# Li-Jinjie/ndp_nmpc_qd

Hardware: AMD Instinct MI355X
Metric: NMPC solves/sec (N=20, 1 RTI iter + downwash MLP) at batch (higher is better)
Workload: dtype f64

## Files before the change

### ndp_nmpc_qd_amd/build.py

```python
import os
import subprocess
import sys
from concurrent.futures import ThreadPoolExecutor

HERE = os.path.dirname(os.path.abspath(__file__))
CSRC = os.path.join(HERE, "csrc")
LIB = os.path.join(HERE, "libndp_nmpc_hip.so")
UNITS = ["ndp_hip.hip", "exchange.hip", "mlp_vjp.hip"]
HEADERS = sorted(f for f in os.listdir(CSRC) if f.endswith((".hpp", ".inc"))) + [os.path.join("..", "..", "include", "ndp_nmpc.h")]
FLAGS = ["--offload-arch=gfx950", "-O3", "-std=c++17", "-mllvm", "-amdgpu-mfma-vgpr-form",
         "-mllvm", "-amdgpu-schedule-relaxed-occupancy=true", "-fPIC"]


def _mtime(p):
    return os.path.getmtime(p) if os.path.exists(p) else -1.0


def build(force=False, verbose=False, out=LIB, extra=()):
    flags = FLAGS + os.environ.get("NDP_EXTRA_HIPCC_FLAGS", "").split() + list(extra)
    odir = os.path.join(HERE, "build", os.path.splitext(os.path.basename(out))[0])
    os.makedirs(odir, exist_ok=True)
    stamp = os.path.join(odir, "flags")
    if not os.path.exists(stamp) or open(stamp).read() != " ".join(flags):
        force = True
    t_hdr = max(_mtime(os.path.join(CSRC, f)) for f in HEADERS)
    objs = [os.path.join(odir, os.path.splitext(u)[0] + ".o") for u in UNITS]
    todo = [(u, o) for u, o in zip(UNITS, objs) if force or _mtime(o) < max(t_hdr, _mtime(os.path.join(CSRC, u)))]

    def compile_unit(job):
        u, o = job
        cmd = ["hipcc"] + flags + ["-c", "-o", o, os.path.join(CSRC, u)]
        if verbose:
            print(" ".join(cmd), flush=True)
        return subprocess.run(cmd, cwd=CSRC).returncode

    if todo:
        if os.path.exists(stamp):
            os.remove(stamp)
        jobs = max(1, min(16, len(todo), int(os.environ.get("MAX_JOBS") or 16)))
        with ThreadPoolExecutor(jobs) as ex:
            failed = [u for (u, _), rc in zip(todo, ex.map(compile_unit, todo)) if rc != 0]
        if failed:
            raise subprocess.CalledProcessError(1, "hipcc " + " ".join(failed))
        with open(stamp, "w") as fh:
            fh.write(" ".join(flags))
    if todo or _mtime(out) < max(_mtime(o) for o in objs):
        cmd = ["hipcc", "-shared", "-o", out] + objs
        if verbose:
            print(" ".join(cmd), flush=True)
        subprocess.check_call(cmd, cwd=CSRC)
    return out


if __name__ == "__main__":
    args = sys.argv[1:]
    out = LIB
    if args[:1] == ["-o"]:
        out, args = os.path.abspath(args[1]), args[2:]
    print(build(force=True, verbose=True, out=out, extra=args))
```

### ndp_nmpc_qd_amd/csrc/kern_args.hpp

```cpp
#pragma once
#include <hip/hip_runtime.h>

#include <stddef.h>

namespace ndp {

struct ThrCfg { double a1, a2, hm, g, R, Q0, Q1, mass; };

struct RingGeom {
    int step, np1;
    __host__ __device__ int ring() const { return step * (np1 - 1) + 1; }
    __host__ __device__ size_t px() const { return (size_t)step * 2 * np1 * 10; }
    __host__ __device__ size_t pu() const { return (size_t)step * 2 * np1 * 4; }
    __host__ __device__ size_t slot(unsigned long long j) const { return (size_t)(j % step) * 2 * np1 + (size_t)((j / step) % np1); }
};

struct RefCfg { int B, N, n_seg; double dt, mass, g, toff; };

struct TickPre {
    RefCfg cf;
    const double *coeff, *tcum, *tseg, *fpt;
    int *seg_hint;
    const double *t;
    double t_all;
    int advance;
    unsigned long long j_new;
    RingGeom rg;
    double *rx, *ru;
    ThrCfg thr;
    double *st;
// ... 10 lines not shown
```

### ndp_nmpc_qd_amd/csrc/ndp_hip.hip

```cpp
#include <hip/hip_runtime.h>
#include <hip/hip_ext.h>

#include <sched.h>
#include <stdio.h>

#include <atomic>
#include <chrono>
#include <condition_variable>
#include <cstdlib>
#include <cstring>
#include <memory>
#include <mutex>
#include <new>
#include <string>
#include <thread>
#include <type_traits>
#include <vector>

#include "wave_gfx950.hpp"
#include "cfg_params.hpp"
#include "cond_qp.hpp"
#include "host.hpp"
#include "mlp_common.hpp"

namespace ndp {

struct BatchPtrs {
    const double *kc;
    const int *tables;
    const double *x0, *xr, *ur;
    const float *f;
    double *X, *U, *u0;
    int *status, *iters;
    double *Xm, *Um;
    double *dbg;
    double *stamps;
    size_t xr_pitch, ur_pitch;
    size_t x0_pitch;
    double *cmd;
    const double *kthr;
    double *thrust_keep;
    double cmd_mass;
    int f_f64;
    signed char *act;
};

struct MlpArgs {
    const float *frag;
    const double *other;
    const double *ego_xy;
    float *force_out;
    double r2;
    int other_stride;
// ... 3 lines not shown
    size_t ego_pitch;
};

struct QueueArgs {
    unsigned *count;
    int *ids;
    unsigned long long *ipm_total;
};

typedef __attribute__((address_space(3))) float *lds_f32;
typedef const __attribute__((address_space(3))) float *lds_cf32;
__device__ __forceinline__ void stage_fragments(const float *__restrict__ fr, lds_f32 dst, int tid, int nthreads);
__device__ __forceinline__ void mlp_tile(lds_cf32 fr, const float zb[3], int lane, float o[3]);
__device__ __forceinline__ bool gate_open(const double *other_inst, const double *ego_xy_inst, double r2);

__device__ __forceinline__ void bind_instance(RtiIo &io, const BatchPtrs &bp, int inst, int N)
{
    const size_t nx = (size_t)(N + 1) * NX, nu = (size_t)N * NU, nf = (size_t)(N + 1) * 3;
    io.x0 = bp.x0 + (size_t)inst * bp.x0_pitch;
    io.xr = bp.xr + inst * bp.xr_pitch;
    io.ur = bp.ur + inst * bp.ur_pitch;
    io.f = bp.f ? bp.f + inst * nf * (bp.f_f64 ? 2 : 1) : nullptr;
    io.f_is_f64 = bp.f_f64;
    io.X = bp.X + inst * nx;
    io.U = bp.U + inst * nu;
    io.Xm = bp.Xm ? bp.Xm + inst * nx : nullptr;
    io.Um = bp.Xm ? bp.Um + inst * nu : nullptr;
    io.u0 = bp.u0 + (size_t)inst * NU;
    io.status = bp.status + inst;
    io.iters = bp.iters + inst;
    io.dbg = bp.dbg;
    io.f_in_lds = 0;
    io.kc = bp.kc;
    io.tables = bp.tables;
    io.stamps = bp.stamps ? bp.stamps + (size_t)inst * NDP_NSTAMP : nullptr;
    io.act = bp.act ? bp.act + (size_t)inst * act_pitch(N) : nullptr;
    if (NDP_RARELY(bp.cmd != nullptr)) {
        io.cmd = bp.cmd + (size_t)inst * NU;
        io.thrust_keep = bp.thrust_keep + inst;
        io.kthr = bp.kthr[inst];
// ... 50 lines not shown
    LateArgs la;
    TickArgs ta;
};
struct SensArgs {
    double *du0 = nullptr, *dU = nullptr, *dX = nullptr;
    int level = 0;
};
struct PSensArgs {
    double *dxr = nullptr, *dur = nullptr, *df = nullptr;
};

struct KernargLate {
    const __attribute__((address_space(4))) unsigned *kp;
    __device__ __forceinline__ KernargLate()
    {
        kp = (const __attribute__((address_space(4))) unsigned *)__builtin_amdgcn_kernarg_segment_ptr();
        asm volatile("" : "+s"(kp));
    }
    template <class T> __device__ __forceinline__ T get(unsigned off) const
    {
        static_assert(sizeof(T) % 4 == 0 && std::is_trivially_copyable<T>::value, "plain words only");
        unsigned w[sizeof(T) / 4];
#pragma unroll
        for (unsigned i = 0; i < sizeof(T) / 4; ++i) w[i] = kp[off / 4 + i];
        T t;
        __builtin_memcpy(&t, w, sizeof(T));
        return t;
    }
};
static_assert(offsetof(KernArgs, P) == 0, "WaveGfx950::late_params reads the parameter block at the start of the argument segment");
static_assert(std::is_standard_layout<KernArgs>::value && std::is_trivially_copyable<KernArgs>::value,
              "KernargLate addresses members of the one kernel argument by offsetof");
#define NDP_TA_LATE(L, f) ((L).template get<decltype(TickArgs::f)>((unsigned)(offsetof(KernArgs, ta) + offsetof(TickArgs, f))))
template <class T> using gptr = __attribute__((address_space(1))) T *;

#ifndef NDP_RTI_ATTR
#define NDP_RTI_ATTR
#endif
template <int NSLOT, int WAVES, bool FUSED, int NC = 0, int PREC = 0, int NRC = (NC ? 1 : 0), int QMODE = 0, bool TICK = false>
__global__ __launch_bounds__(64 * WAVES) NDP_RTI_ATTR void rti_kernel(KernArgs ka)
{
    constexpr bool SENS = false, PSENS = false;
    const SensArgs sa{};
    const PSensArgs pa{};
    extern __shared__ __attribute__((aligned(16))) double smem[];
    __shared__ unsigned wg_done;
#include "rti_kernel_body.inc"
}

template <int WAVES, bool FUSED, int NC, int QMODE>
__global__ __launch_bounds__(64 * WAVES) void rti_sens_kernel(KernArgs ka, SensArgs sa)
{
    constexpr int NSLOT = 3, PREC = 0, NRC = NC ? 1 : 0;
    constexpr bool TICK = false, SENS = true, PSENS = false;
    const PSensArgs pa{};
    extern __shared__ __attribute__((aligned(16))) double smem[];
    __shared__ unsigned wg_done;
#include "rti_kernel_body.inc"
}

template <int WAVES, bool FUSED, int NC, int QMODE>
__global__ __launch_bounds__(64 * WAVES) void rti_psens_kernel(KernArgs ka, SensArgs sa, PSensArgs pa)
{
    constexpr int NSLOT = 3, PREC = 0, NRC = NC ? 1 : 0;
    constexpr bool TICK = false, SENS = true, PSENS = true;
    extern __shared__ __attribute__((aligned(16))) double smem[];
    __shared__ unsigned wg_done;
#include "rti_kernel_body.inc"
}

struct VjpArgs {
    const double *gu0, *gX, *gU;
    double *gx0, *gxr, *gur, *gf;
};
template <int NC>
__global__ __launch_bounds__(256) void rti_vjp_kernel(KernArgs ka, VjpArgs va)
{
    extern __shared__ __attribute__((aligned(16))) double smem[];
    const RtiParams &P = ka.P;
    const int waves = (int)(blockDim.x >> 6), wave = (int)(threadIdx.x >> 6);
    const int inst = __builtin_amdgcn_readfirstlane((int)blockIdx.x * waves + wave);
    if (inst >= ka.B) return;
    const int N = NC ? NC : P.N;
    RtiIo io;
    bind_instance(io, ka.bp, inst, N);
    const int lpw = NC ? ((lds_doubles(NC) + 1) & ~1) : ka.lds_per_wave;
    WaveGfx950::lds_ptr lds = (WaveGfx950::lds_ptr)(smem + (size_t)wave * lpw);
    using Prog = RtiWave<WaveGfx950, 3, NC, true, NC ? 1 : 0>;
    const size_t i = (size_t)inst, nx = (size_t)(N + 1) * NX, nu = (size_t)N * NU, nf = (size_t)(N + 1) * 3;
    const VjpIo vo{va.gu0 ? va.gu0 + i * NU : nullptr, va.gX ? va.gX + i * nx : nullptr, va.gU ? va.gU + i * nu : nullptr,
                   va.gx0 ? va.gx0 + i * NX : nullptr, va.gxr ? va.gxr + i * nx : nullptr, va.gur ? va.gur + i * nu : nullptr,
                   va.gf ? va.gf + i * nf : nullptr};
    typename Prog::InBuf inb;
    double x0v;
    Prog::issue_first(P, io, inb, x0v);
    Prog::template run<false, true, false, false, true>(P, io, lds, inb, x0v, nullptr, nullptr, &vo);
}

template <int NC>
__global__ __launch_bounds__(256) void rti_wvjp_kernel(KernArgs ka, VjpArgs va, double *gmodel)
{
    extern __shared__ __attribute__((aligned(16))) double smem[];
    const RtiParams &P = ka.P;
    const int waves = (int)(blockDim.x >> 6), wave = (int)(threadIdx.x >> 6);
    const int inst = __builtin_amdgcn_readfirstlane((int)blockIdx.x * waves + wave);
    if (inst >= ka.B) return;
    const int N = NC ? NC : P.N;
    RtiIo io;
    bind_instance(io, ka.bp, inst, N);
    const int lpw = NC ? ((lds_doubles(NC) + 1) & ~1) : ka.lds_per_wave;
    WaveGfx950::lds_ptr lds = (WaveGfx950::lds_ptr)(smem + (size_t)wave * lpw);
    using Prog = RtiWave<WaveGfx950, 3, NC, true, NC ? 1 : 0>;
    const size_t i = (size_t)inst, nx = (size_t)(N + 1) * NX, nu = (size_t)N * NU, nf = (size_t)(N + 1) * 3;
    const VjpIo vo{va.gu0 ? va.gu0 + i * NU : nullptr, va.gX ? va.gX + i * nx : nullptr, va.gU ? va.gU + i * nu : nullptr,
                   va.gx0 ? va.gx0 + i * NX : nullptr, va.gxr ? va.gxr + i * nx : nullptr, va.gur ? va.gur + i * nu : nullptr,
                   va.gf ? va.gf + i * nf : nullptr};
    typename Prog::InBuf inb;
    double x0v;
    Prog::issue_first(P, io, inb, x0v);
    Prog::template run<false, true, false, false, true, true>(P, io, lds, inb, x0v, nullptr, nullptr, &vo, gmodel + i * 16);
}

__global__ void mfma_probe_kernel(const double *a, const double *b, const double *c, double *d)
// ... 1647 lines not shown
    if (phase == 1) {
        if (N != 20) return K40_PROD;
        if (tick) return fused ? K20F_PROD_TICK : K20_PROD_TICK;
        return fused ? K20F_PROD : K20_PROD;
    }
    if (ref && W == 4) {
        if (tick) return fused ? K20F_TICK : K20_TICK;
        return fused ? K20F : prefetched ? K20_LATE : K20;
    }
    if (ref && W == 2) return fused ? K20F_W2 : K20_W2;
    if (N == 40 && h->cfg.n_rti == 2 && W == 2 && !fused) return K40;
    if (fused) return (RtiId)(K3F_4 + wi);
    return (RtiId)((slots_for(N) <= 3 ? K3_4 : K5_4) + wi);
}

static void launch_kern(const ndp_handle *h, RtiId id, hipStream_t s, KernArgs &ka, SensArgs &sa, hipEvent_t start = nullptr,
                        hipEvent_t stop = nullptr)
{
    const RtiKern &k = k_rti[id];
    h->rti_launched.fetch_or(1ull << id, std::memory_order_relaxed);
    const dim3 grid((h->cfg.batch + k.waves - 1) / k.waves), block(64 * k.waves);
    const size_t shm = (size_t)h->lds_per_wave * sizeof(double) * k.waves;
    PSensArgs pa{h->dPSensXr, h->dPSensUr, h->dPSensF};
    void *args[] = {&ka, &sa, &pa};
    if (start || stop) (void)hipExtLaunchKernel(k.fn, grid, block, args, shm, s, start, stop, 0);
    else (void)hipLaunchKernel(k.fn, grid, block, args, shm, s);
}

static int launch_rti(ndp_handle *h, const double *d_x0, const double *d_xr, const double *d_ur, const float *d_f,
                      double *d_u0, double *d_dbg, hipStream_t s, const Neigh *nb = nullptr, const StepOut *so = nullptr,
                      bool prefetched = false)
{
    int *d_status = so && so->status ? so->status : h->dStatus, *d_iters = so && so->iters ? so->iters : h->dIters;
    h->lastStatus = d_status; h->lastIters = d_iters;
    BatchPtrs bp{h->dKC, h->dTables, d_x0, d_xr, d_ur, d_f, h->dX, h->dU, d_u0, d_status, d_iters,
                 so ? so->Xm : nullptr, so ? so->Um : nullptr, d_dbg, h->dStamps,
                 so && so->xr_pitch ? so->xr_pitch : (size_t)(h->cfg.N + 1) * NX, so && so->ur_pitch ? so->ur_pitch : (size_t)h->cfg.N * NU, (size_t)NX,
                 so ? so->cmd : nullptr, so ? so->kthr : nullptr, so ? so->thrust_keep : nullptr, h->cfg.mass, so && so->f_f64 ? 1 : 0,
                 h->dAct};
    const bool fused = nb && nb->other;
    MlpArgs ma{fused ? h->dFrag : nullptr, fused ? nb->other : nullptr, fused ? nb->ego_xy : nullptr, h->dForce,
               h->cfg.r_horiz * h->cfg.r_horiz, fused ? nb->stride : NX, fused ? nb->index : nullptr, fused ? peer_mapped(nb->other) : 0,
               fused && nb->pitch ? nb->pitch : (size_t)(h->cfg.N + 1) * (fused ? nb->stride : NX), fused && nb->ego_pitch ? nb->ego_pitch : (size_t)2};
    QueueArgs qa{h->dQctr, h->dQids, reinterpret_cast<unsigned long long *>(h->dQctr + 16)};
    LateArgs la{prefetched ? h->dProto : nullptr, {h->dForceAB[0], h->dForceAB[1]}, h->prefetch_timeout_us,
                h->pf_groups_rti, h->pf_ntiles};
    KernArgs ka{h->P, bp, h->cfg.batch, h->lds_per_wave, ma, qa, la, so && so->tick ? *so->tick : TickArgs{}};
    SensArgs sa{h->dSensU0, h->sens_level >= 2 ? h->dSensU : nullptr, h->sens_level >= 2 ? h->dSensX : nullptr, h->sens_level};
    const bool tick1 = so && so->tick;
    const int pr = h->cfg.qp_precision;
    const bool q = h->use_queue && !d_dbg && !prefetched;
    h->last_step_tracked = false;
    if (h->track_steps) {
        hipStreamCaptureStatus cs = hipStreamCaptureStatusNone;
        if (hipStreamIsCapturing(s, &cs) != hipSuccess) { (void)hipGetLastError(); cs = hipStreamCaptureStatusNone; }
        if (cs != hipStreamCaptureStatusNone) {
            h->err = "tracked control steps (ndp_track_steps) cannot be launched on a stream that is being captured: switch tracking off "
                     "and order the exchange through the stream (ndp_xchg_begin's after_stream)";
            return -15;
        }
    }
    int rc = begin_timing(h, s, 0, true);
    if (rc) return rc;
    const bool ext_timing = h->timing_open && !q && !pr && !(so && so->done) && !h->track_steps;
    if (h->timing_open && !ext_timing) NDP_HIP(h, hipEventRecord(h->events.back().a, s));
    if (pr && fused) { h->err = "qp_precision != 0 supports f / no disturbance only (run ndp_downwash first)"; return -12; }
    hipEvent_t stop = nullptr;
    if (so && so->done) stop = so->done;
    else if (h->track_steps) { stop = h->stepDone[++h->step_seq & 3]; h->last_step_tracked = true; }
    if (h->sens_level > 0 && (prefetched || tick1)) { h->err = "launch_rti: the late-force and tick forms have no sensitivity kernel"; return -2; }
    launch_kern(h, rti_pick(h, fused, tick1, prefetched, q ? 1 : 0), s, ka, sa, ext_timing ? h->events.back().a : nullptr,
                ext_timing ? h->events.back().b : q || pr ? nullptr : stop);
    if (ext_timing) h->timing_open = false;
    NDP_HIP(h, hipGetLastError());
    if (q) {
        KernArgs kc = ka;
// ... 1311 lines not shown
    const size_t B = c.batch;
    if (!h->dVjp) {
        NDP_HIP(h, hipMalloc((void **)&h->dVjp, (nxs(h) + nus(h) + B * NU) * 8));
        NDP_HIP(h, hipMalloc((void **)&h->dVjpSt, B * 2 * 4));
        NDP_HIP(h, hipMalloc((void **)&h->dVjpAct, act_bytes(h)));
    }
    double *X = h->dVjp, *U = X + nxs(h), *u0 = U + nus(h);
    int *st = h->dVjpSt, *it = st + B;
    hipStream_t s = g.s;
    NDP_HIP(h, hipMemcpyAsync(X, d_X_lin, nxs(h) * 8, hipMemcpyDeviceToDevice, s));
    NDP_HIP(h, hipMemcpyAsync(U, d_U_lin, nus(h) * 8, hipMemcpyDeviceToDevice, s));
    if (d_act_lin) NDP_HIP(h, hipMemcpyAsync(h->dVjpAct, d_act_lin, act_bytes(h), hipMemcpyDeviceToDevice, s));
    else NDP_HIP(h, hipMemsetAsync(h->dVjpAct, 0, act_bytes(h), s));
    BatchPtrs bp{h->dKC, h->dTables, (const double *)d_x0, (const double *)d_xr, (const double *)d_ur, (const float *)d_f, X, U,
                 d_u0_check ? (double *)d_u0_check : u0, d_status_check ? (int *)d_status_check : st, it, nullptr, nullptr, nullptr, nullptr,
                 (size_t)(c.N + 1) * NX, (size_t)c.N * NU, (size_t)NX, nullptr, nullptr, nullptr, c.mass, 0, h->dVjpAct};
    KernArgs ka{h->P, bp, (int)B, h->lds_per_wave, MlpArgs{}, QueueArgs{}, LateArgs{}, TickArgs{}};
    VjpArgs va{(const double *)d_gu0, (const double *)d_gX, (const double *)d_gU, (double *)d_gx0, (double *)d_gxr, (double *)d_gur,
               (double *)d_gf};
    const int W = h->waves;
    const void *fn = model ? (c.N == 20 ? (const void *)rti_wvjp_kernel<20> : (const void *)rti_wvjp_kernel<0>)
                           : (c.N == 20 ? (const void *)rti_vjp_kernel<20> : (const void *)rti_vjp_kernel<0>);
    double *gm = (double *)d_gmodel;
    void *args[] = {&ka, &va, &gm};
    NDP_HIP(h, hipLaunchKernel(fn, dim3((unsigned)((B + W - 1) / W)), dim3(64 * W), args, (size_t)h->lds_per_wave * sizeof(double) * W, s));
    NDP_HIP(h, hipGetLastError());
    return g.noted(0);
}

int ndp_step_vjp_device(ndp_handle *h, const void *d_x0, const void *d_xr, const void *d_ur, const void *d_f,
                        const void *d_X_lin, const void *d_U_lin, const void *d_act_lin,
                        const void *d_gu0, const void *d_gX, const void *d_gU,
                        void *d_gx0, void *d_gxr, void *d_gur, void *d_gf, void *d_u0_check, void *d_status_check, void *stream)
{
    return step_vjp(h, d_x0, d_xr, d_ur, d_f, d_X_lin, d_U_lin, d_act_lin, d_gu0, d_gX, d_gU, d_gx0, d_gxr, d_gur, d_gf, d_u0_check,
                    d_status_check, stream, false, nullptr);
}

int ndp_step_vjp_model_device(ndp_handle *h, const void *d_x0, const void *d_xr, const void *d_ur, const void *d_f,
// ... 84 lines not shown
```

### ndp_nmpc_qd_amd/csrc/rti_kernel_body.inc

```
    static_assert(!(FUSED && QMODE == 2), "the consumer reads the force the producer left in global memory");
    static_assert(!TICK || (QMODE <= 1 && NC > 0 && PREC == 0), "the one-launch tick exists for the compile-time horizon's in-place and producer forms");
#ifndef NDP_NO_KERNARG_WARM
    {
        typedef const __attribute__((address_space(4))) unsigned *kptr;
        kptr kp = (kptr)__builtin_amdgcn_kernarg_segment_ptr();
        unsigned acc = 0;
#pragma unroll
        for (unsigned o = 0; o < (unsigned)sizeof(KernArgs); o += 64) acc |= kp[o / 4];
        asm volatile("" : : "s"(acc));
    }
#endif
    const RtiParams &P = ka.P;
    const BatchPtrs &bp = ka.bp;
    const MlpArgs &ma = ka.ma;
    const QueueArgs &qa = ka.qa;
    const int B = ka.B;
    const int wave = (int)(threadIdx.x >> 6);
    if (!FUSED && (QMODE == 0 || QMODE == 3) && ka.la.proto) {
        if (threadIdx.x == 0) wg_done = 0;
        __syncthreads();
    }
    int inst_raw = __builtin_amdgcn_readfirstlane((int)blockIdx.x * WAVES + wave);
    if (QMODE == 2) {
        const int n = (int)*qa.count;
        if (inst_raw >= n) return;
        inst_raw = __builtin_amdgcn_readfirstlane(qa.ids[inst_raw]);
    }
    const bool active = inst_raw < B;
    if (!FUSED && !active) return;
    const int inst = active ? inst_raw : B - 1;
    const int N = NC ? NC : P.N;
    const size_t nf = (size_t)(N + 1) * 3;
    RtiIo io;
    bind_instance(io, bp, inst, N);
    if (NSLOT <= 3 && (QMODE == 0 || QMODE == 3)) io.ipm_ctr = qa.ipm_total;
    if (NSLOT <= 3 && QMODE != 2 && blockIdx.x == 0 && threadIdx.x == 0 && qa.ipm_total)
        __hip_atomic_fetch_add(qa.ipm_total + 1, 1ull, __ATOMIC_RELAXED, __HIP_MEMORY_SCOPE_AGENT);
    if (!FUSED && (QMODE == 0 || QMODE == 3) && ka.la.proto) {
        const LateArgs &la = ka.la;
        const unsigned long long t = la.proto[PF_RTI_C2] / la.groups_rti + 1;
        const unsigned g = blockIdx.x % la.groups_rti;
        const unsigned np1 = (unsigned)N + 1, row0 = (unsigned)inst * np1;
        io.f_late = la.F[t & 1] + (size_t)inst * nf;
        io.late_flag = la.proto + PF_EPOCH + (t & 1) * la.ntiles + row0 / 32;
        io.late_flag2 = la.proto + PF_EPOCH + (t & 1) * la.ntiles + (row0 + np1 - 1) / 32;
        io.late_want = t;
        io.late_ready = la.proto[PF_MLP_DONE] >= t ? 1 : 0;
        io.late_timeout_us = la.timeout_us;
        io.late_missed = reinterpret_cast<int *>(la.proto + PF_MISSED);
        io.late_slow = reinterpret_cast<int *>(la.proto + PF_SLOW);
        io.late_cnt = reinterpret_cast<unsigned *>(la.proto + PF_RTI_C1 + PF_STRIDE * g);
        io.late_done_word = la.proto + PF_RTI_C2;
        io.late_gsize = pf_group_size(gridDim.x, la.groups_rti, g);
        io.late_group = (void *)((size_t)(unsigned)(size_t)(__attribute__((address_space(3))) unsigned *)&wg_done + 1);
        const int left = B - (int)blockIdx.x * WAVES;
        io.late_group_size = (unsigned)(left < WAVES ? left : WAVES);
    }
    const int lpw = NC ? ((lds_doubles(NC) + 1) & ~1) : ka.lds_per_wave;
    WaveGfx950::lds_ptr lds = (WaveGfx950::lds_ptr)(smem + (size_t)wave * lpw);
    using WB = std::conditional_t<PREC == 3, WaveGfx950F32, std::conditional_t<PREC == 4, WaveGfx950BF16, WaveGfx950>>;
    using Prog = RtiWave<WB, NSLOT, NC, true, NRC, (PREC >= 3 ? 0 : PREC), QMODE == 3, (PREC == 5 ? 1 : (PREC == 6 ? 2 : 0))>;
    if (NDP_RARELY(io.stamps && (threadIdx.x & 63u) == 0)) {
        io.stamps[12] = (double)__builtin_amdgcn_s_memrealtime();
        io.stamps[14] = (double)__builtin_amdgcn_s_memtime();
    }
    int orow = inst;
    bool wg_nb = true;
    if (FUSED && ma.other_index) {
        int any = 0;
#pragma unroll
        for (int w = 0; w < WAVES; ++w) {
            const int iw = (int)blockIdx.x * WAVES + w;
            any |= (ma.other_index[iw < B ? iw : B - 1] >= 0) ? 1 : 0;
        }
        orow = __builtin_amdgcn_readfirstlane(ma.other_index[inst]);
        asm volatile("" : : "s"(orow));
        wg_nb = __builtin_amdgcn_readfirstlane(any) != 0;
    }
    const bool advance = TICK && ka.ta.advance != 0;
    TickEarly te;
    if (TICK && NDP_RARELY(io.stamps && (threadIdx.x & 63u) == 0)) io.stamps[16] = (double)__builtin_amdgcn_s_memtime();
    if (TICK && advance) {
        te = tick_early(ka.ta, inst, FUSED && wg_nb ? orow : -1, (int)(threadIdx.x & 63u));
        __builtin_amdgcn_sched_barrier(0);
    }
    if (TICK && NDP_RARELY(io.stamps && (threadIdx.x & 63u) == 0)) io.stamps[22] = (double)__builtin_amdgcn_s_memtime();
    typename Prog::InBuf inb;
    double x0v;
    Prog::issue_first(P, io, inb, x0v);
    __builtin_amdgcn_sched_barrier(0);
    if (TICK && NDP_RARELY(io.stamps && (threadIdx.x & 63u) == 0)) io.stamps[23] = (double)__builtin_amdgcn_s_memtime();
    double x_new[10], u_new[4], nb_new[6], seg_fill = 0.0, seg_cfill = 0.0;
    int seg_refill = 0;
    if (TICK && !(FUSED && wg_nb) && advance) {
        tick_arrived(te);
        seg_fill = tick_new_point(ka.ta, te, inst, (int)(threadIdx.x & 63u), active, x_new, u_new, nb_new, seg_refill, seg_cfill, io.stamps);
#pragma unroll
        for (int i = 0; i < 10; ++i) io.xrN[i] = x_new[i];
        io.have_xrN = 1;
    }
    if (FUSED && !wg_nb) {
        if (!active) return;
        const int lane = (int)(threadIdx.x & 63u);
        const LdsMap m = make_map(N);
// ... 115 lines not shown
```

### ndp_nmpc_qd_amd/csrc/rti_wave.hpp

```cpp
#pragma once
#define NDP_RARELY(x) (__builtin_expect_with_probability(!!(x), 0, 0.9999))

#ifndef NDP_D
#define NDP_D inline
#endif
#if defined(__clang__)
#define NDP_UNROLL_STAGES _Pragma("unroll UNROLL_STAGES")
#define NDP_UNROLL_SWEEP _Pragma("unroll UNROLL_SWEEP")
#define NDP_KEEP_LOOP _Pragma("unroll 1")
#else
#define NDP_UNROLL_STAGES
#define NDP_UNROLL_SWEEP
#define NDP_KEEP_LOOP
#endif
#ifdef NDP_FINE_STAMPS
#define NDP_FINE(x) x
#else
#define NDP_FINE(x)
#endif
#ifndef NDP_HD
#define NDP_HD inline
#endif

namespace ndp {
// ... 348 lines not shown

    static NDP_D void load_tables(const int *g, Tables &T)
    {
        lane_preds(T);
        vi lane = W::lane();
        for_each_int(T, [&](int i, vi &fld) { fld = W::gldi(g, lane * 4 + ((i >> 2) * 256 + (i & 3))); });
    }

    static constexpr int NMAXS = (64 * NSLOT + 3) / 7;
    static constexpr int RX = ((NMAXS + 1) * NX + 63) / 64, RU = (NMAXS * NU + 63) / 64, RF = ((NMAXS + 1) * 3 + 63) / 64;

    struct InBuf { vd xr[RX], xi[RX], ur[RU], ui[RU], f[RF], kc; };

    static NDP_D void issue_inputs(const RtiParams &P, const RtiIo &io, InBuf &b, bool first)
    {
        const int N = horizon(P);
        vi lane = lane_it();
        const int nx = (N + 1) * NX, nu = N * NU, nf = (N + 1) * 3;
        const bool have_f = P.use_fd && io.f && !io.f_in_lds;
        for (int t = 0; t < RX; ++t) {
            vi i = W::imin(lane + 64 * t, nx - 1);
            b.xr[t] = W::gldu(io.xr, i);
            b.xi[t] = first ? W::gldu(io.X, i) : vd(0.0);
        }
        for (int t = 0; t < RU; ++t) {
            vi i = W::imin(lane + 64 * t, nu - 1);
            b.ur[t] = W::gldu(io.ur, i);
            b.ui[t] = first ? W::gldu(io.U, i) : vd(0.0);
        }
        for (int t = 0; t < RF; ++t) {
            vi i = W::imin(lane + 64 * t, nf - 1);
            b.f[t] = have_f ? (NDP_RARELY(io.f_is_f64 != 0) ? W::gldu(reinterpret_cast<const double *>(io.f), i) : W::gldfu(io.f, i)) : vd(0.0);
        }
        b.kc = first ? W::gldu(io.kc, W::imin(lane, KC_HOST - 1)) : vd(0.0);
    }

    static NDP_D void commit_inputs(const RtiParams &P, const LdsMap &m, const InBuf &b, lp lds, bool first, const RtiIo &io)
    {
        const int N = horizon(P);
        vi lane = lane_it();
        const int nx = (N + 1) * NX, nu = N * NU, nf = (N + 1) * 3;
        for (int t = 0; t < RX; ++t) {
            vi i = W::imin(lane + 64 * t, nx - 1);
            W::st(lds, i + m.TXR, b.xr[t]);
// ... 1141 lines not shown

    static NDP_D void stamp(const RtiIo &io, const LdsMap &m, int idx)
    {
        if (NDP_RARELY(io.dbg)) {
            vd t = W::clock();
            W::gst(io.dbg, W::lane() * 0 + (m.total + idx), t, W::lane() == 0);
        }
        if (NDP_RARELY(io.stamps)) {
            vd t = W::clock();
            W::gst(io.stamps, W::lane() * 0 + idx, t, W::lane() == 0);
        }
    }

    static NDP_D void issue_first(const RtiParams &P, const RtiIo &io, InBuf &inb, vd &x0v)
    {
        vi lane = W::lane();
        x0v = W::gldu(io.x0, W::imin(lane, NX - 1));
        RtiIo g = io;
        g.f_in_lds = 0;
        issue_inputs(P, g, inb, true);
    }

    static NDP_D void run(const RtiParams &P, const RtiIo &io, lp lds)
    {
        InBuf inb;
        vd x0v;
        issue_first(P, io, inb, x0v);
        run<false>(P, io, lds, inb, x0v);
    }


    template <bool DEFER, bool IPM_RARE = false, bool SENS = false, bool PSENS = false, bool VJP = false, bool WVJP = false>
    static NDP_D bool run(const RtiParams &P, const RtiIo &io, lp lds, InBuf &inb, vd x0v, const SensIo *sens = nullptr,
                          const PSensIo *psens = nullptr, const VjpIo *vjp = nullptr, double *gmodel = nullptr)
    {
// ... 589 lines not shown
```

### ndp_nmpc_qd_amd/csrc/wave_gfx950.hpp

```cpp
#pragma once
#include <hip/hip_runtime.h>

#define NDP_D __device__ __forceinline__
#define NDP_HD __host__ __device__ inline

namespace ndp {

struct RtiParams;
struct LdsMap;

struct WaveGfx950 {
    using vd = double;
    using vi = int;
    using vb = bool;
    struct vd4 { double r[4]; };
    using md = double;
    using md4 = vd4;
    static constexpr bool packed_k = false, delta_ok = true, has_mma4 = true;
    static NDP_D md to_m(vd a) { return a; }
    static NDP_D vd to_d(md a) { return a; }
    static NDP_D md4 mzero4() { return zero4(); }
    static NDP_D md mavg(md a, md b) { return (a + b) * 0.5; }
    static NDP_D md msel(vb p, md a, md b) { return p ? a : b; }
    static NDP_D vi lcol(vi lane) { return lane & 15; }
// ... 30 lines not shown
    {
        __builtin_amdgcn_fence(__ATOMIC_RELEASE, "wavefront");
        __builtin_amdgcn_wave_barrier();
        __builtin_amdgcn_fence(__ATOMIC_ACQUIRE, "wavefront");
    }

    static NDP_D vd gld(const double *g, vi off, vb p) { return p ? g[off] : 0.0; }
    static NDP_D vd gldf(const float *g, vi off, vb p) { return p ? (double)g[off] : 0.0; }
    static NDP_D vd gldu(const double *g, vi off) { return g[off]; }
    static NDP_D vd gldfu(const float *g, vi off) { return (double)g[off]; }
    static NDP_D vi gldi(const int *g, vi off) { return g[off]; }
    template <class T>
    static NDP_D const __attribute__((address_space(4))) T *late_params(const T &)
    {
        typedef const __attribute__((address_space(4))) T *kptr;
        kptr base = (kptr)__builtin_amdgcn_kernarg_segment_ptr();
        asm volatile("" : "+s"(base));
        return base;
    }
    static NDP_D vi gld_i8(const signed char *g, vi off) { return (int)g[off]; }
    static NDP_D vi d2i(vd a) { return (int)a; }
    static NDP_D vd i2d(vi a) { return (double)a; }
    static NDP_D void gst_i8(signed char *g, vi off, vi v, vb p) { if (p) g[off] = (signed char)v; }
    static NDP_D vi imin(vi a, vi b) { return a < b ? a : b; }
    static NDP_D void gst(double *g, vi off, vd v, vb p) { if (p) g[off] = v; }
    static NDP_D void gst2(double *a, double *b, vi i, int n, vd v) { (i < n ? a + i : b + (i - n))[0] = v; }
    static NDP_D void gsti(int *g, int v) { if (g && lane() == 0) *g = v; }
    static NDP_D void cmd_store(double *cmd, double *keep, double k, double mass, vi idx, vd v, vb p)
    {
        if (p) {
            if (idx == 3) {
// ... 203 lines not shown
```

### ndp_nmpc_qd_amd/isa_inspect.py

```python
import os
import re
import struct
import subprocess
import tempfile

LLVM = "/opt/rocm/lib/llvm/bin"
MAGIC = b"__CLANG_OFFLOAD_BUNDLE__"


def device_code_objects(so_path, arch="gfx950"):
    data = open(so_path, "rb").read()
    out = []
    i = data.find(MAGIC)
    while i >= 0:
        n = struct.unpack_from("<Q", data, i + len(MAGIC))[0]
        off = i + len(MAGIC) + 8
        for _ in range(n):
            o, sz, tl = struct.unpack_from("<QQQ", data, off)
            off += 24
            triple = data[off:off + tl].decode()
            off += tl
            if arch in triple and sz:
                out.append(data[i + o:i + o + sz])
        i = data.find(MAGIC, off)
# ... 47 lines not shown
        return self._home[symbol]

    def disassemble(self, symbol):
        path = self.code_object_of(symbol)
        txt = subprocess.run([os.path.join(LLVM, "llvm-objdump"), "-d", "--no-show-raw-insn", f"--disassemble-symbols={symbol}", path],
                             check=True, capture_output=True, text=True).stdout
        out = []
        for ln in txt.split("\n"):
            s = ln.split("//")[0].strip()
            if not s or s.endswith(":") or s.startswith(("Disassembly", path, "/")) or "file format" in s:
                continue
            out.append(s)
        return out


def rti_kernel_name(nslot, waves, fused, nc=0, prec=0, nrc=None, qmode=0, tick=False):
    nrc = (1 if nc else 0) if nrc is None else nrc
    return (f"_ZN3ndp10rti_kernelILi{nslot}ELi{waves}ELb{1 if fused else 0}ELi{nc}ELi{prec}ELi{nrc}ELi{qmode}ELb{1 if tick else 0}EEEvNS_8KernArgsE")


def epoch_store_is_ordered(insns):
    ep = [i for i, s in enumerate(insns) if s.startswith("global_store_dwordx2")]
    if not ep:
        return False, "no epoch store (global_store_dwordx2) found"
    for e in ep:
        rows = [i for i in range(e) if insns[i].startswith("global_store_dword ") or insns[i].startswith("global_store_dword\t")]
        if not rows:
            return False, "no row store in front of the epoch store"
        between = insns[rows[-1] + 1:e]
        if not any(s.startswith("s_waitcnt") and re.search(r"vmcnt\(0\)", s) for s in between):
            return False, "no s_waitcnt vmcnt(0) between the last row store and the epoch store: " + " | ".join(between[-6:])
    return True, f"{len(ep)} epoch store(s), each behind s_waitcnt vmcnt(0)"
```

Baseline: 46.26 million.

## Preload hot kernel arguments into SGPRs and issue first input loads earlier

```diff
diff --git a/ndp_nmpc_qd_amd/build.py b/ndp_nmpc_qd_amd/build.py
--- a/ndp_nmpc_qd_amd/build.py
+++ b/ndp_nmpc_qd_amd/build.py
@@ -10,6 +10,7 @@
 HEADERS = sorted(f for f in os.listdir(CSRC) if f.endswith((".hpp", ".inc"))) + [os.path.join("..", "..", "include", "ndp_nmpc.h")]
 FLAGS = ["--offload-arch=gfx950", "-O3", "-std=c++17", "-mllvm", "-amdgpu-mfma-vgpr-form",
          "-mllvm", "-amdgpu-schedule-relaxed-occupancy=true", "-fPIC"]
+UNIT_FLAGS = {"ndp_hip.hip": ["-mllvm", "-amdgpu-kernarg-preload-count=8"]}
 
 
 def _mtime(p):
@@ -21,7 +22,8 @@
     odir = os.path.join(HERE, "build", os.path.splitext(os.path.basename(out))[0])
     os.makedirs(odir, exist_ok=True)
     stamp = os.path.join(odir, "flags")
-    if not os.path.exists(stamp) or open(stamp).read() != " ".join(flags):
+    flags_key = " ".join(flags + [f"[{u}: {' '.join(f)}]" for u, f in sorted(UNIT_FLAGS.items())])
+    if not os.path.exists(stamp) or open(stamp).read() != flags_key:
         force = True
     t_hdr = max(_mtime(os.path.join(CSRC, f)) for f in HEADERS)
     objs = [os.path.join(odir, os.path.splitext(u)[0] + ".o") for u in UNITS]
@@ -29,7 +31,7 @@
 
     def compile_unit(job):
         u, o = job
-        cmd = ["hipcc"] + flags + ["-c", "-o", o, os.path.join(CSRC, u)]
+        cmd = ["hipcc"] + flags + UNIT_FLAGS.get(u, []) + ["-c", "-o", o, os.path.join(CSRC, u)]
         if verbose:
             print(" ".join(cmd), flush=True)
         return subprocess.run(cmd, cwd=CSRC).returncode
@@ -43,7 +45,7 @@
         if failed:
             raise subprocess.CalledProcessError(1, "hipcc " + " ".join(failed))
         with open(stamp, "w") as fh:
-            fh.write(" ".join(flags))
+            fh.write(flags_key)
     if todo or _mtime(out) < max(_mtime(o) for o in objs):
         cmd = ["hipcc", "-shared", "-o", out] + objs
         if verbose:
diff --git a/ndp_nmpc_qd_amd/csrc/kern_args.hpp b/ndp_nmpc_qd_amd/csrc/kern_args.hpp
--- a/ndp_nmpc_qd_amd/csrc/kern_args.hpp
+++ b/ndp_nmpc_qd_amd/csrc/kern_args.hpp
@@ -14,6 +14,18 @@
     __host__ __device__ size_t pu() const { return (size_t)step * 2 * np1 * 4; }
     __host__ __device__ size_t slot(unsigned long long j) const { return (size_t)(j % step) * 2 * np1 + (size_t)((j / step) % np1); }
 };
+
+struct HotArgs {
+    const double *x0, *xr, *ur;
+    double *X, *U;
+    unsigned xr_pitch, ur_pitch;
+    int B;
+};
+enum { NDP_HOT_ARGS = 8, NDP_HOT_BYTES = 56, NDP_HOT_DWORDS = NDP_HOT_BYTES / 4 };
+static_assert(sizeof(HotArgs) == NDP_HOT_BYTES && NDP_HOT_DWORDS <= 14, "13 preloaded dwords, the block behind them 8-byte aligned");
+#define NDP_HOT_PARAMS const double *hot_x0, const double *hot_xr, const double *hot_ur, double *hot_X, double *hot_U, \
+                       unsigned hot_xr_pitch, unsigned hot_ur_pitch, int hot_B
+#define NDP_HOT_VALUE HotArgs{hot_x0, hot_xr, hot_ur, hot_X, hot_U, hot_xr_pitch, hot_ur_pitch, hot_B}
 
 struct RefCfg { int B, N, n_seg; double dt, mass, g, toff; };
 
diff --git a/ndp_nmpc_qd_amd/csrc/ndp_hip.hip b/ndp_nmpc_qd_amd/csrc/ndp_hip.hip
--- a/ndp_nmpc_qd_amd/csrc/ndp_hip.hip
+++ b/ndp_nmpc_qd_amd/csrc/ndp_hip.hip
@@ -36,7 +36,6 @@
     double *dbg;
     double *stamps;
     size_t xr_pitch, ur_pitch;
-    size_t x0_pitch;
     double *cmd;
     const double *kthr;
     double *thrust_keep;
@@ -70,16 +69,21 @@
 __device__ __forceinline__ void mlp_tile(lds_cf32 fr, const float zb[3], int lane, float o[3]);
 __device__ __forceinline__ bool gate_open(const double *other_inst, const double *ego_xy_inst, double r2);
 
+__device__ __forceinline__ void bind_hot(RtiIo &io, const HotArgs &ha, int inst, int N)
+{
+    const size_t nx = (size_t)(N + 1) * NX, nu = (size_t)N * NU;
+    io.x0 = ha.x0 + (size_t)inst * NX;
+    io.xr = ha.xr + (size_t)inst * ha.xr_pitch;
+    io.ur = ha.ur + (size_t)inst * ha.ur_pitch;
+    io.X = ha.X + inst * nx;
+    io.U = ha.U + inst * nu;
+}
+
 __device__ __forceinline__ void bind_instance(RtiIo &io, const BatchPtrs &bp, int inst, int N)
 {
     const size_t nx = (size_t)(N + 1) * NX, nu = (size_t)N * NU, nf = (size_t)(N + 1) * 3;
-    io.x0 = bp.x0 + (size_t)inst * bp.x0_pitch;
-    io.xr = bp.xr + inst * bp.xr_pitch;
-    io.ur = bp.ur + inst * bp.ur_pitch;
     io.f = bp.f ? bp.f + inst * nf * (bp.f_f64 ? 2 : 1) : nullptr;
     io.f_is_f64 = bp.f_f64;
-    io.X = bp.X + inst * nx;
-    io.U = bp.U + inst * nu;
     io.Xm = bp.Xm ? bp.Xm + inst * nx : nullptr;
     io.Um = bp.Xm ? bp.Um + inst * nu : nullptr;
     io.u0 = bp.u0 + (size_t)inst * NU;
@@ -160,7 +164,7 @@
     const __attribute__((address_space(4))) unsigned *kp;
     __device__ __forceinline__ KernargLate()
     {
-        kp = (const __attribute__((address_space(4))) unsigned *)__builtin_amdgcn_kernarg_segment_ptr();
+        kp = (const __attribute__((address_space(4))) unsigned *)__builtin_amdgcn_kernarg_segment_ptr() + NDP_HOT_DWORDS;
         asm volatile("" : "+s"(kp));
     }
     template <class T> __device__ __forceinline__ T get(unsigned off) const
@@ -174,9 +178,9 @@
         return t;
     }
 };
-static_assert(offsetof(KernArgs, P) == 0, "WaveGfx950::late_params reads the parameter block at the start of the argument segment");
+static_assert(alignof(KernArgs) == 8 && offsetof(KernArgs, P) == 0, "WaveGfx950::late_params reads the parameter block at the start of the KernArgs block (NDP_HOT_BYTES into the argument segment)");
 static_assert(std::is_standard_layout<KernArgs>::value && std::is_trivially_copyable<KernArgs>::value,
-              "KernargLate addresses members of the one kernel argument by offsetof");
+              "KernargLate addresses members of the KernArgs argument by offsetof");
 #define NDP_TA_LATE(L, f) ((L).template get<decltype(TickArgs::f)>((unsigned)(offsetof(KernArgs, ta) + offsetof(TickArgs, f))))
 template <class T> using gptr = __attribute__((address_space(1))) T *;
 
@@ -184,7 +188,7 @@
 #define NDP_RTI_ATTR
 #endif
 template <int NSLOT, int WAVES, bool FUSED, int NC = 0, int PREC = 0, int NRC = (NC ? 1 : 0), int QMODE = 0, bool TICK = false>
-__global__ __launch_bounds__(64 * WAVES) NDP_RTI_ATTR void rti_kernel(KernArgs ka)
+__global__ __launch_bounds__(64 * WAVES) NDP_RTI_ATTR void rti_kernel(NDP_HOT_PARAMS, KernArgs ka)
 {
     constexpr bool SENS = false, PSENS = false;
     const SensArgs sa{};
@@ -195,7 +199,7 @@
 }
 
 template <int WAVES, bool FUSED, int NC, int QMODE>
-__global__ __launch_bounds__(64 * WAVES) void rti_sens_kernel(KernArgs ka, SensArgs sa)
+__global__ __launch_bounds__(64 * WAVES) void rti_sens_kernel(NDP_HOT_PARAMS, KernArgs ka, SensArgs sa)
 {
     constexpr int NSLOT = 3, PREC = 0, NRC = NC ? 1 : 0;
     constexpr bool TICK = false, SENS = true, PSENS = false;
@@ -206,7 +210,7 @@
 }
 
 template <int WAVES, bool FUSED, int NC, int QMODE>
-__global__ __launch_bounds__(64 * WAVES) void rti_psens_kernel(KernArgs ka, SensArgs sa, PSensArgs pa)
+__global__ __launch_bounds__(64 * WAVES) void rti_psens_kernel(NDP_HOT_PARAMS, KernArgs ka, SensArgs sa, PSensArgs pa)
 {
     constexpr int NSLOT = 3, PREC = 0, NRC = NC ? 1 : 0;
     constexpr bool TICK = false, SENS = true, PSENS = true;
@@ -220,15 +224,17 @@
     double *gx0, *gxr, *gur, *gf;
 };
 template <int NC>
-__global__ __launch_bounds__(256) void rti_vjp_kernel(KernArgs ka, VjpArgs va)
+__global__ __launch_bounds__(256) void rti_vjp_kernel(NDP_HOT_PARAMS, KernArgs ka, VjpArgs va)
 {
     extern __shared__ __attribute__((aligned(16))) double smem[];
     const RtiParams &P = ka.P;
     const int waves = (int)(blockDim.x >> 6), wave = (int)(threadIdx.x >> 6);
     const int inst = __builtin_amdgcn_readfirstlane((int)blockIdx.x * waves + wave);
-    if (inst >= ka.B) return;
+    const HotArgs ha = NDP_HOT_VALUE;
+    if (inst >= ha.B) return;
     const int N = NC ? NC : P.N;
     RtiIo io;
+    bind_hot(io, ha, inst, N);
     bind_instance(io, ka.bp, inst, N);
     const int lpw = NC ? ((lds_doubles(NC) + 1) & ~1) : ka.lds_per_wave;
     WaveGfx950::lds_ptr lds = (WaveGfx950::lds_ptr)(smem + (size_t)wave * lpw);
@@ -244,15 +250,17 @@
 }
 
 template <int NC>
-__global__ __launch_bounds__(256) void rti_wvjp_kernel(KernArgs ka, VjpArgs va, double *gmodel)
+__global__ __launch_bounds__(256) void rti_wvjp_kernel(NDP_HOT_PARAMS, KernArgs ka, VjpArgs va, double *gmodel)
 {
     extern __shared__ __attribute__((aligned(16))) double smem[];
     const RtiParams &P = ka.P;
     const int waves = (int)(blockDim.x >> 6), wave = (int)(threadIdx.x >> 6);
     const int inst = __builtin_amdgcn_readfirstlane((int)blockIdx.x * waves + wave);
-    if (inst >= ka.B) return;
+    const HotArgs ha = NDP_HOT_VALUE;
+    if (inst >= ha.B) return;
     const int N = NC ? NC : P.N;
     RtiIo io;
+    bind_hot(io, ha, inst, N);
     bind_instance(io, ka.bp, inst, N);
     const int lpw = NC ? ((lds_doubles(NC) + 1) & ~1) : ka.lds_per_wave;
     WaveGfx950::lds_ptr lds = (WaveGfx950::lds_ptr)(smem + (size_t)wave * lpw);
@@ -1930,6 +1938,13 @@
     return (RtiId)((slots_for(N) <= 3 ? K3_4 : K5_4) + wi);
 }
 
+static HotArgs hot_args(const KernArgs &ka)
+{
+    return HotArgs{ka.bp.x0, ka.bp.xr, ka.bp.ur, ka.bp.X, ka.bp.U, (unsigned)ka.bp.xr_pitch, (unsigned)ka.bp.ur_pitch, ka.B};
+}
+static bool hot_fits(const KernArgs &ka) { return ((ka.bp.xr_pitch | ka.bp.ur_pitch) >> 32) == 0; }
+#define NDP_HOT_ARGV(ha) &(ha).x0, &(ha).xr, &(ha).ur, &(ha).X, &(ha).U, &(ha).xr_pitch, &(ha).ur_pitch, &(ha).B
+
 static void launch_kern(const ndp_handle *h, RtiId id, hipStream_t s, KernArgs &ka, SensArgs &sa, hipEvent_t start = nullptr,
                         hipEvent_t stop = nullptr)
 {
@@ -1938,7 +1953,8 @@
     const dim3 grid((h->cfg.batch + k.waves - 1) / k.waves), block(64 * k.waves);
     const size_t shm = (size_t)h->lds_per_wave * sizeof(double) * k.waves;
     PSensArgs pa{h->dPSensXr, h->dPSensUr, h->dPSensF};
-    void *args[] = {&ka, &sa, &pa};
+    HotArgs ha = hot_args(ka);
+    void *args[] = {NDP_HOT_ARGV(ha), &ka, &sa, &pa};
     if (start || stop) (void)hipExtLaunchKernel(k.fn, grid, block, args, shm, s, start, stop, 0);
     else (void)hipLaunchKernel(k.fn, grid, block, args, shm, s);
 }
@@ -1951,7 +1967,7 @@
     h->lastStatus = d_status; h->lastIters = d_iters;
     BatchPtrs bp{h->dKC, h->dTables, d_x0, d_xr, d_ur, d_f, h->dX, h->dU, d_u0, d_status, d_iters,
                  so ? so->Xm : nullptr, so ? so->Um : nullptr, d_dbg, h->dStamps,
-                 so && so->xr_pitch ? so->xr_pitch : (size_t)(h->cfg.N + 1) * NX, so && so->ur_pitch ? so->ur_pitch : (size_t)h->cfg.N * NU, (size_t)NX,
+                 so && so->xr_pitch ? so->xr_pitch : (size_t)(h->cfg.N + 1) * NX, so && so->ur_pitch ? so->ur_pitch : (size_t)h->cfg.N * NU,
                  so ? so->cmd : nullptr, so ? so->kthr : nullptr, so ? so->thrust_keep : nullptr, h->cfg.mass, so && so->f_f64 ? 1 : 0,
                  h->dAct};
     const bool fused = nb && nb->other;
@@ -1976,6 +1992,7 @@
             return -15;
         }
     }
+    if (!hot_fits(ka)) { h->err = "launch_rti: the pitch of xr or ur does not fit 32 bits"; return -2; }
     int rc = begin_timing(h, s, 0, true);
     if (rc) return rc;
     const bool ext_timing = h->timing_open && !q && !pr && !(so && so->done) && !h->track_steps;
@@ -3317,7 +3334,7 @@
     else NDP_HIP(h, hipMemsetAsync(h->dVjpAct, 0, act_bytes(h), s));
     BatchPtrs bp{h->dKC, h->dTables, (const double *)d_x0, (const double *)d_xr, (const double *)d_ur, (const float *)d_f, X, U,
                  d_u0_check ? (double *)d_u0_check : u0, d_status_check ? (int *)d_status_check : st, it, nullptr, nullptr, nullptr, nullptr,
-                 (size_t)(c.N + 1) * NX, (size_t)c.N * NU, (size_t)NX, nullptr, nullptr, nullptr, c.mass, 0, h->dVjpAct};
+                 (size_t)(c.N + 1) * NX, (size_t)c.N * NU, nullptr, nullptr, nullptr, c.mass, 0, h->dVjpAct};
     KernArgs ka{h->P, bp, (int)B, h->lds_per_wave, MlpArgs{}, QueueArgs{}, LateArgs{}, TickArgs{}};
     VjpArgs va{(const double *)d_gu0, (const double *)d_gX, (const double *)d_gU, (double *)d_gx0, (double *)d_gxr, (double *)d_gur,
                (double *)d_gf};
@@ -3325,7 +3342,8 @@
     const void *fn = model ? (c.N == 20 ? (const void *)rti_wvjp_kernel<20> : (const void *)rti_wvjp_kernel<0>)
                            : (c.N == 20 ? (const void *)rti_vjp_kernel<20> : (const void *)rti_vjp_kernel<0>);
     double *gm = (double *)d_gmodel;
-    void *args[] = {&ka, &va, &gm};
+    HotArgs ha = hot_args(ka);
+    void *args[] = {NDP_HOT_ARGV(ha), &ka, &va, &gm};
     NDP_HIP(h, hipLaunchKernel(fn, dim3((unsigned)((B + W - 1) / W)), dim3(64 * W), args, (size_t)h->lds_per_wave * sizeof(double) * W, s));
     NDP_HIP(h, hipGetLastError());
     return g.noted(0);
diff --git a/ndp_nmpc_qd_amd/csrc/rti_kernel_body.inc b/ndp_nmpc_qd_amd/csrc/rti_kernel_body.inc
--- a/ndp_nmpc_qd_amd/csrc/rti_kernel_body.inc
+++ b/ndp_nmpc_qd_amd/csrc/rti_kernel_body.inc
@@ -1,25 +1,24 @@
     static_assert(!(FUSED && QMODE == 2), "the consumer reads the force the producer left in global memory");
     static_assert(!TICK || (QMODE <= 1 && NC > 0 && PREC == 0), "the one-launch tick exists for the compile-time horizon's in-place and producer forms");
+    const HotArgs ha = NDP_HOT_VALUE;
 #ifndef NDP_NO_KERNARG_WARM
+    typedef const __attribute__((address_space(4))) unsigned *kwarm_ptr;
+    constexpr unsigned KWARM = ((unsigned)NDP_HOT_BYTES + (unsigned)sizeof(KernArgs) + 63u) / 64u;
+    unsigned kwarm[KWARM];
     {
-        typedef const __attribute__((address_space(4))) unsigned *kptr;
-        kptr kp = (kptr)__builtin_amdgcn_kernarg_segment_ptr();
-        unsigned acc = 0;
-#pragma unroll
-        for (unsigned o = 0; o < (unsigned)sizeof(KernArgs); o += 64) acc |= kp[o / 4];
-        asm volatile("" : : "s"(acc));
-    }
+        kwarm_ptr kp = (kwarm_ptr)__builtin_amdgcn_kernarg_segment_ptr();
+#pragma unroll
+        for (unsigned o = 0; o < KWARM; ++o) kwarm[o] = kp[o * 16];
+    }
+    __builtin_amdgcn_sched_barrier(0);
 #endif
     const RtiParams &P = ka.P;
     const BatchPtrs &bp = ka.bp;
     const MlpArgs &ma = ka.ma;
     const QueueArgs &qa = ka.qa;
-    const int B = ka.B;
+    const int B = ha.B;
     const int wave = (int)(threadIdx.x >> 6);
-    if (!FUSED && (QMODE == 0 || QMODE == 3) && ka.la.proto) {
-        if (threadIdx.x == 0) wg_done = 0;
-        __syncthreads();
-    }
+    constexpr bool LATE_FORM = !FUSED && (QMODE == 0 || QMODE == 3);
     int inst_raw = __builtin_amdgcn_readfirstlane((int)blockIdx.x * WAVES + wave);
     if (QMODE == 2) {
         const int n = (int)*qa.count;
@@ -27,11 +26,33 @@
         inst_raw = __builtin_amdgcn_readfirstlane(qa.ids[inst_raw]);
     }
     const bool active = inst_raw < B;
-    if (!FUSED && !active) return;
+    if (!FUSED && !active) {
+        if (LATE_FORM && ka.la.proto) __syncthreads();
+        return;
+    }
     const int inst = active ? inst_raw : B - 1;
     const int N = NC ? NC : P.N;
     const size_t nf = (size_t)(N + 1) * 3;
     RtiIo io;
+    bind_hot(io, ha, inst, N);
+    using WB = std::conditional_t<PREC == 3, WaveGfx950F32, std::conditional_t<PREC == 4, WaveGfx950BF16, WaveGfx950>>;
+    using Prog = RtiWave<WB, NSLOT, NC, true, NRC, (PREC >= 3 ? 0 : PREC), QMODE == 3, (PREC == 5 ? 1 : (PREC == 6 ? 2 : 0))>;
+    typename Prog::InBuf inb;
+    double x0v;
+    Prog::issue_first_rows(N, io, inb, x0v);
+    __builtin_amdgcn_sched_barrier(0);
+#ifndef NDP_NO_KERNARG_WARM
+    {
+        unsigned acc = 0;
+#pragma unroll
+        for (unsigned o = 0; o < KWARM; ++o) acc |= kwarm[o];
+        asm volatile("" : : "s"(acc));
+    }
+#endif
+    if (LATE_FORM && ka.la.proto) {
+        if (threadIdx.x == 0) wg_done = 0;
+        __syncthreads();
+    }
     bind_instance(io, bp, inst, N);
     if (NSLOT <= 3 && (QMODE == 0 || QMODE == 3)) io.ipm_ctr = qa.ipm_total;
     if (NSLOT <= 3 && QMODE != 2 && blockIdx.x == 0 && threadIdx.x == 0 && qa.ipm_total)
@@ -58,8 +79,6 @@
     }
     const int lpw = NC ? ((lds_doubles(NC) + 1) & ~1) : ka.lds_per_wave;
     WaveGfx950::lds_ptr lds = (WaveGfx950::lds_ptr)(smem + (size_t)wave * lpw);
-    using WB = std::conditional_t<PREC == 3, WaveGfx950F32, std::conditional_t<PREC == 4, WaveGfx950BF16, WaveGfx950>>;
-    using Prog = RtiWave<WB, NSLOT, NC, true, NRC, (PREC >= 3 ? 0 : PREC), QMODE == 3, (PREC == 5 ? 1 : (PREC == 6 ? 2 : 0))>;
     if (NDP_RARELY(io.stamps && (threadIdx.x & 63u) == 0)) {
         io.stamps[12] = (double)__builtin_amdgcn_s_memrealtime();
         io.stamps[14] = (double)__builtin_amdgcn_s_memtime();
@@ -85,9 +104,7 @@
         __builtin_amdgcn_sched_barrier(0);
     }
     if (TICK && NDP_RARELY(io.stamps && (threadIdx.x & 63u) == 0)) io.stamps[22] = (double)__builtin_amdgcn_s_memtime();
-    typename Prog::InBuf inb;
-    double x0v;
-    Prog::issue_first(P, io, inb, x0v);
+    Prog::issue_first_rest(P, io, inb);
     __builtin_amdgcn_sched_barrier(0);
     if (TICK && NDP_RARELY(io.stamps && (threadIdx.x & 63u) == 0)) io.stamps[23] = (double)__builtin_amdgcn_s_memtime();
     double x_new[10], u_new[4], nb_new[6], seg_fill = 0.0, seg_cfill = 0.0;
diff --git a/ndp_nmpc_qd_amd/csrc/rti_wave.hpp b/ndp_nmpc_qd_amd/csrc/rti_wave.hpp
--- a/ndp_nmpc_qd_amd/csrc/rti_wave.hpp
+++ b/ndp_nmpc_qd_amd/csrc/rti_wave.hpp
@@ -386,10 +386,14 @@
 
     static NDP_D void issue_inputs(const RtiParams &P, const RtiIo &io, InBuf &b, bool first)
     {
-        const int N = horizon(P);
+        issue_rows(horizon(P), io, b, first);
+        issue_rest(P, io, b, first);
+    }
+
+    static NDP_D void issue_rows(const int N, const RtiIo &io, InBuf &b, bool first)
+    {
         vi lane = lane_it();
-        const int nx = (N + 1) * NX, nu = N * NU, nf = (N + 1) * 3;
-        const bool have_f = P.use_fd && io.f && !io.f_in_lds;
+        const int nx = (N + 1) * NX, nu = N * NU;
         for (int t = 0; t < RX; ++t) {
             vi i = W::imin(lane + 64 * t, nx - 1);
             b.xr[t] = W::gldu(io.xr, i);
@@ -400,6 +404,14 @@
             b.ur[t] = W::gldu(io.ur, i);
             b.ui[t] = first ? W::gldu(io.U, i) : vd(0.0);
         }
+    }
+
+    static NDP_D void issue_rest(const RtiParams &P, const RtiIo &io, InBuf &b, bool first)
+    {
+        const int N = horizon(P);
+        vi lane = lane_it();
+        const int nf = (N + 1) * 3;
+        const bool have_f = P.use_fd && io.f && !io.f_in_lds;
         for (int t = 0; t < RF; ++t) {
             vi i = W::imin(lane + 64 * t, nf - 1);
             b.f[t] = have_f ? (NDP_RARELY(io.f_is_f64 != 0) ? W::gldu(reinterpret_cast<const double *>(io.f), i) : W::gldfu(io.f, i)) : vd(0.0);
@@ -1571,11 +1583,20 @@
 
     static NDP_D void issue_first(const RtiParams &P, const RtiIo &io, InBuf &inb, vd &x0v)
     {
+        issue_first_rows(horizon(P), io, inb, x0v);
+        issue_first_rest(P, io, inb);
+    }
+    static NDP_D void issue_first_rows(const int N, const RtiIo &io, InBuf &inb, vd &x0v)
+    {
         vi lane = W::lane();
         x0v = W::gldu(io.x0, W::imin(lane, NX - 1));
+        issue_rows(N, io, inb, true);
+    }
+    static NDP_D void issue_first_rest(const RtiParams &P, const RtiIo &io, InBuf &inb)
+    {
         RtiIo g = io;
         g.f_in_lds = 0;
-        issue_inputs(P, g, inb, true);
+        issue_rest(P, g, inb, true);
     }
 
     static NDP_D void run(const RtiParams &P, const RtiIo &io, lp lds)
diff --git a/ndp_nmpc_qd_amd/csrc/wave_gfx950.hpp b/ndp_nmpc_qd_amd/csrc/wave_gfx950.hpp
--- a/ndp_nmpc_qd_amd/csrc/wave_gfx950.hpp
+++ b/ndp_nmpc_qd_amd/csrc/wave_gfx950.hpp
@@ -1,5 +1,7 @@
 #pragma once
 #include <hip/hip_runtime.h>
+
+#include "kern_args.hpp"
 
 #define NDP_D __device__ __forceinline__
 #define NDP_HD __host__ __device__ inline
@@ -68,7 +70,7 @@
     static NDP_D const __attribute__((address_space(4))) T *late_params(const T &)
     {
         typedef const __attribute__((address_space(4))) T *kptr;
-        kptr base = (kptr)__builtin_amdgcn_kernarg_segment_ptr();
+        kptr base = (kptr)((const __attribute__((address_space(4))) char *)__builtin_amdgcn_kernarg_segment_ptr() + NDP_HOT_BYTES);
         asm volatile("" : "+s"(base));
         return base;
     }
diff --git a/ndp_nmpc_qd_amd/isa_inspect.py b/ndp_nmpc_qd_amd/isa_inspect.py
--- a/ndp_nmpc_qd_amd/isa_inspect.py
+++ b/ndp_nmpc_qd_amd/isa_inspect.py
@@ -85,9 +85,12 @@
         return out
 
 
+RTI_PARAMS = "PKdS2_S2_PdS3_jjiNS_8KernArgsE"
+
+
 def rti_kernel_name(nslot, waves, fused, nc=0, prec=0, nrc=None, qmode=0, tick=False):
     nrc = (1 if nc else 0) if nrc is None else nrc
-    return (f"_ZN3ndp10rti_kernelILi{nslot}ELi{waves}ELb{1 if fused else 0}ELi{nc}ELi{prec}ELi{nrc}ELi{qmode}ELb{1 if tick else 0}EEEvNS_8KernArgsE")
+    return (f"_ZN3ndp10rti_kernelILi{nslot}ELi{waves}ELb{1 if fused else 0}ELi{nc}ELi{prec}ELi{nrc}ELi{qmode}ELb{1 if tick else 0}EEEv" + RTI_PARAMS)
 
 
 def epoch_store_is_ordered(insns):
```

New measurement: 46.17 million. No clear change (-0.2%).
